# nvidia-cosmos/cosmos-curate

Hardware: AMD Instinct MI355X
Metric: clips/sec + embedded frames/sec, 1080p30 H.264, 1/2/4/8 MI355X (higher is better)
Workload: dtype bf16; 1 GPU; split_pipeline 1xMI355X: HIP NV12->RGB/resize + CLIP-ViT-B/32 MFMA bf16 (decode seam excluded: no librocdecode in image); model=vit_b32, frames_per_clip=21, src=1080p30 NV12 in HBM, resolution=224, parallelism=dp1

## Files before the change

cosmos_curate_amd/csrc/cc_gemm.hip:

```cpp

#include <hip/hip_runtime.h>

#include "cc_common.hpp"
#include "cc_gemm_plan.hpp"
#include "cc_timing.hpp"

namespace {

typedef __attribute__((ext_vector_type(8))) __bf16 bf16x8;
typedef __attribute__((ext_vector_type(4))) float f32x4;

constexpr int BM = cc::GEMM_T128, BN = cc::GEMM_T128, BK = cc::GEMM_BK;
constexpr int WM = 64, WN = 64;
constexpr int FRAG = 16;
constexpr int MFR = WM / FRAG;
constexpr int NFR = WN / FRAG;

__device__ __forceinline__ unsigned short f32_to_bf16_rne(float v) {
  union {
    float f;
    unsigned int u;
  } cv{v};
  unsigned int lsb = (cv.u >> 16) & 1;
  return (unsigned short)((cv.u + 0x7fffu + lsb) >> 16);
}

template <int ACT>
__device__ __forceinline__ float cc_act(float v) {
  if constexpr (ACT == 1)
    return v * __builtin_amdgcn_rcpf(1.0f + __expf(-1.702f * v));
  if constexpr (ACT == 2) {
    float z = 0.7978845608028654f * (v + 0.044715f * v * v * v);
    float t = 1.0f - 2.0f * __builtin_amdgcn_rcpf(__expf(2.0f * z) + 1.0f);
    return 0.5f * v * (1.0f + t);
  }
  if constexpr (ACT == 3)
    return 0.5f * v * (1.0f + erff(v * 0.70710678f));
  return v;
}

__device__ __forceinline__ int xcd_remap(int orig, int nwg) {
  int q = nwg >> 3, r = nwg & 7;
  int xcd = orig & 7, lid = orig >> 3;
  return (xcd < r ? xcd * (q + 1) : r * (q + 1) + (xcd - r) * q) + lid;
}

template <int CHUNKS>
__device__ __forceinline__ void stage_rows(const __bf16* __restrict__ src,
                                           long ld, long row0, long row_limit,
                                           long k0, __bf16* lds_base,
                                           int lane) {
  const int lrow8 = lane >> 3;
  const int slot = lane & 7;
  const int gk16 = slot ^ lrow8;
#pragma unroll
  for (int j = 0; j < CHUNKS; j++) {
    long grow = row0 + j * 8 + lrow8;
    grow = grow < 0 ? 0 : (grow >= row_limit ? row_limit - 1 : grow);
    const __bf16* gptr = src + grow * ld + k0 + (long)gk16 * 8;
    __builtin_amdgcn_global_load_lds(
        (const __attribute__((address_space(1))) unsigned int*)gptr,
        (__attribute__((address_space(3))) unsigned int*)(lds_base + j * 8 * BK),
        16, 0, 0);
  }
}

__device__ __forceinline__ bf16x8 frag_read(const __bf16* tile, int row,
                                            int k16) {
  int slot = k16 ^ (row & 7);
  return *(const bf16x8*)(tile + (long)row * BK + slot * 8);
}

template <int ACT, bool HAS_BIAS, bool HAS_RES, bool LN_IN>
__global__ __launch_bounds__(256, 2) void k_gemm_bf16(
    const __bf16* __restrict__ A, const __bf16* __restrict__ B,
    void* __restrict__ C, const float* __restrict__ bias,
    const __bf16* __restrict__ residual, long M, long N, long K, long lda,
    long ldr, int c_is_bf16, int nbx, int nwg, int do_remap,
    const float* __restrict__ colsum, const float2* __restrict__ murstd) {
  __shared__ __bf16 lds[2 * (BM + BN) * BK];
#define AS(b) (lds + (b) * (BM * BK))
#define BS(b) (lds + 2 * (BM * BK) + (b) * (BN * BK))

  const int tid = threadIdx.x;
  const int lane = tid & 63;
  const int wid = tid >> 6;
  const int waveM = wid >> 1, waveN = wid & 1;

  int orig = blockIdx.x;
  if (do_remap) orig = xcd_remap(orig, nwg);
  const long bm = (long)(orig / nbx) * BM;
  const long bn = (long)(orig % nbx) * BN;

  const long arow0 = bm + 32 * wid;
  const long brow0 = bn + 32 * wid;

  f32x4 acc[MFR][NFR] = {};

  const long KT = K / BK;
  stage_rows<4>(A, lda, arow0, M, 0, AS(0) + 32 * wid * BK, lane);
  stage_rows<4>(B, K, brow0, N, 0, BS(0) + 32 * wid * BK, lane);

  const int arow_frag = waveM * WM + (lane & 15);
  const int brow_frag = waveN * WN + (lane & 15);
  int buf = 0;
  for (long kt = 0; kt < KT; ++kt) {
    asm volatile("s_waitcnt vmcnt(0)" ::: "memory");
    __syncthreads();
    const __bf16* At = AS(buf);
    const __bf16* Bt = BS(buf);
    bf16x8 afrag[2][MFR], bfrag[2][NFR];
#pragma unroll
    for (int g = 0; g < 2; g++) {
      const int k16 = (g << 2) + (lane >> 4);
#pragma unroll
      for (int m = 0; m < MFR; m++)
        afrag[g][m] = frag_read(At, arow_frag + m * FRAG, k16);
#pragma unroll
      for (int n = 0; n < NFR; n++)
        bfrag[g][n] = frag_read(Bt, brow_frag + n * FRAG, k16);
    }
    if (kt + 1 < KT) {
      const long k0 = (kt + 1) * BK;
      stage_rows<4>(A, lda, arow0, M, k0, AS(buf ^ 1) + 32 * wid * BK, lane);
      stage_rows<4>(B, K, brow0, N, k0, BS(buf ^ 1) + 32 * wid * BK, lane);
    }
#pragma unroll
    for (int g = 0; g < 2; g++)
#pragma unroll
      for (int m = 0; m < MFR; m++)
#pragma unroll
        for (int n = 0; n < NFR; n++)
          acc[m][n] = __builtin_amdgcn_mfma_f32_16x16x32_bf16(
              afrag[g][m], bfrag[g][n], acc[m][n], 0, 0, 0);
    buf ^= 1;
  }

  const long crow_base = bm + waveM * WM + 4 * (lane >> 4);
  const long ccol_base = bn + waveN * WN + (lane & 15);
  const bool interior = (bm + BM <= M) && (bn + BN <= N);
  if (interior) {
#pragma unroll
    for (int m = 0; m < MFR; m++) {
      float2 mr[4] = {};
      if constexpr (LN_IN) {
#pragma unroll
        for (int r = 0; r < 4; r++) mr[r] = murstd[crow_base + m * FRAG + r];
      }
#pragma unroll
      for (int n = 0; n < NFR; n++) {
        const long col = ccol_base + n * FRAG;
        float bval = 0.0f;
        if constexpr (HAS_BIAS) bval = bias[col];
        if constexpr (LN_IN) {
          const float sval = colsum[col];
#pragma unroll
          for (int r = 0; r < 4; r++)
            acc[m][n][r] = mr[r].y * (acc[m][n][r] - mr[r].x * sval);
        }
        float rv[4];
        if constexpr (HAS_RES) {
#pragma unroll
          for (int r = 0; r < 4; r++)
            rv[r] = (float)residual[(crow_base + m * FRAG + r) * ldr + col];
        }
#pragma unroll
        for (int r = 0; r < 4; r++) {
          const long row = crow_base + m * FRAG + r;
          float v = cc_act<ACT>(acc[m][n][r] + bval);
          if constexpr (HAS_RES) v += rv[r];
          if (c_is_bf16)
            ((unsigned short*)C)[row * N + col] = f32_to_bf16_rne(v);
          else
            ((float*)C)[row * N + col] = v;
        }
      }
    }
    return;
  }
#pragma unroll
  for (int m = 0; m < MFR; m++) {
#pragma unroll
    for (int n = 0; n < NFR; n++) {
      const long col = ccol_base + n * FRAG;
      if (col >= N) continue;
      float bval = 0.0f;
      if constexpr (HAS_BIAS) bval = bias[col];
#pragma unroll
      for (int r = 0; r < 4; r++) {
        const long row = crow_base + m * FRAG + r;
        if (row >= M) continue;
        if constexpr (LN_IN) {
          const float2 mr = murstd[row];
          acc[m][n][r] = mr.y * (acc[m][n][r] - mr.x * colsum[col]);
        }
        float v = cc_act<ACT>(acc[m][n][r] + bval);
        if constexpr (HAS_RES) v += (float)residual[row * ldr + col];
        if (c_is_bf16)
          ((unsigned short*)C)[row * N + col] = f32_to_bf16_rne(v);
        else
          ((float*)C)[row * N + col] = v;
      }
    }
  }
#undef AS
#undef BS
}

constexpr int BM2 = cc::GEMM_T256, BN2 = cc::GEMM_T256;
constexpr int WM2 = 128, WN2 = 64;
constexpr int MFR2 = WM2 / FRAG;
constexpr int NFR2 = WN2 / FRAG;

constexpr int LN_TAB = BM2 * 4;

template <int CTRL>
__device__ __forceinline__ float dpp_add(float v) {
  const int o = __builtin_amdgcn_update_dpp(0, __builtin_bit_cast(int, v),
                                            CTRL, 0xf, 0xf, false);
  return v + __builtin_bit_cast(float, o);
}
__device__ __forceinline__ float sum8(float v) {
  return dpp_add<0x141>(dpp_add<0x4e>(dpp_add<0xb1>(v)));
}

template <int ACT, bool HAS_BIAS, bool HAS_RES, bool EPI_STAGED, bool LN_IN,
          bool STATS>
__global__ __launch_bounds__(512, 1) void k_gemm_bf16_t256(
    const __bf16* __restrict__ A, const __bf16* __restrict__ B,
    void* __restrict__ C, const float* __restrict__ bias,
    const __bf16* __restrict__ residual, long M, long N, long K,
    int c_is_bf16, int nbx, int nwg, int order_mode,
    const float* __restrict__ colsum, const float2* __restrict__ murstd,
    float2* __restrict__ stats) {
  static_assert(!STATS || HAS_RES, "the stats epilogue is the residual one");
  __shared__ __bf16 lds[2 * (BM2 + BN2) * BK + (LN_IN ? 2 * LN_TAB : 0)];
#define LNTAB(b) ((float*)(lds + 2 * (BM2 + BN2) * BK + (b) * LN_TAB))
#define STAGE_LN2(b)                                                        \
  do {                                                                      \
    if constexpr (LN_IN) {                                                  \
      const long r = bm + (tid >> 1);                                       \
      const float* g = (const float*)(murstd + (r < M ? r : M - 1)) +       \
                       (tid & 1);                                           \
      __builtin_amdgcn_global_load_lds(                                     \
          (const __attribute__((address_space(1))) unsigned int*)g,         \
          (__attribute__((address_space(3))) unsigned int*)(LNTAB(b) +      \
                                                            wid * 64),      \
          4, 0, 0);                                                         \
    }                                                                       \
  } while (0)
#define A2T(b) (lds + (b) * (BM2 * BK))
#define B2T(b) (lds + 2 * (BM2 * BK) + (b) * (BN2 * BK))
  const int tid = threadIdx.x;
  const int lane = tid & 63;
  const int wid = tid >> 6;
  const int waveM = wid >> 2, waveN = wid & 3;
  const long KT = K / BK;
  const long srow = wid * 16;
  const int arow_base = waveM * WM2 + (lane & 15);
  const int brow_base = waveN * WN2 + (lane & 15);
  bf16x8 bfragT[NFR2][2];
  bf16x8 afrag[2][2];

#define STAGE_A2(t, h)                                                      \
  stage_rows<2>(A, K, bm + (h) * 128 + srow, M, (t) * BK,                   \
                A2T((t) & 1) + ((h) * 128 + srow) * BK, lane)
#define STAGE_B2(t, h)                                                      \
  stage_rows<2>(B, K, bn + (h) * 128 + srow, N, (t) * BK,                   \
                B2T((t) & 1) + ((h) * 128 + srow) * BK, lane)

  const int tiles = (nwg + (int)gridDim.x - 1) / (int)gridDim.x;
  long bm, bn;
  {
    int orig = (int)blockIdx.x;
    if (order_mode == 1) orig = xcd_remap(orig, nwg);
    bm = (long)(orig / nbx) * BM2;
    bn = (long)(orig % nbx) * BN2;
  }
  STAGE_LN2(0);
  STAGE_A2(0, 0);
  STAGE_A2(0, 1);
  STAGE_B2(0, 0);
  STAGE_B2(0, 1);
  STAGE_B2(1, 0);
  STAGE_B2(1, 1);

  for (int rep = 0; rep < tiles; rep++) {
    if ((int)blockIdx.x + rep * (int)gridDim.x >= nwg) break;
    f32x4 acc[MFR2][NFR2] = {};
    asm volatile("s_waitcnt vmcnt(0)" ::: "memory");
    __builtin_amdgcn_s_barrier();

#define PHASE_MFMA2(q)                                                      \
  do {                                                                      \
    asm volatile("s_waitcnt lgkmcnt(0)" ::: "memory");                      \
     \
     \
     \
     \
     \
     \
     \
     \
     \
     \
    __builtin_amdgcn_sched_group_barrier(0x8 , 2, 0);               \
    _Pragma("unroll") for (int gi = 0; gi < 6; gi++) {                      \
      __builtin_amdgcn_sched_group_barrier(0x100 , 1, 0);        \
      __builtin_amdgcn_sched_group_barrier(0x8 , 2, 0);             \
      __builtin_amdgcn_sched_group_barrier(0x10 , 1, 0);            \
    }                                                                       \
    _Pragma("unroll") for (int g = 0; g < 2; g++) {                         \
      _Pragma("unroll") for (int m = 0; m < 2; m++) {                       \
        _Pragma("unroll") for (int n = 0; n < NFR2; n++) {                  \
          acc[2 * (q) + m][n] = __builtin_amdgcn_mfma_f32_16x16x32_bf16(    \
              afrag[m][g], bfragT[n][g], acc[2 * (q) + m][n], 0, 0, 0);     \
        }                                                                   \
      }                                                                     \
    }                                                                       \
  } while (0)

#define READ_A2(At, q)                                                      \
  _Pragma("unroll") for (int g = 0; g < 2; g++) {                           \
    const int k16 = (g << 2) + (lane >> 4);                                 \
    _Pragma("unroll") for (int m = 0; m < 2; m++) afrag[m][g] =             \
        frag_read(At, arow_base + (q) * 32 + m * FRAG, k16);                \
  }

#define READ_B2(Bt)                                                         \
  _Pragma("unroll") for (int g = 0; g < 2; g++) {                           \
    const int k16 = (g << 2) + (lane >> 4);                                 \
    _Pragma("unroll") for (int n = 0; n < NFR2; n++) bfragT[n][g] =         \
        frag_read(Bt, brow_base + n * FRAG, k16);                           \
  }

#define KTILE2(t)                                                           \
  do {                                                                      \
    const __bf16* At = A2T((t) & 1);                                        \
    const __bf16* Bt = B2T((t) & 1);                                        \
     \
     \
     \
    asm volatile("s_waitcnt vmcnt(4)" ::: "memory");                        \
    READ_B2(Bt);                                                            \
    READ_A2(At, 0);                                                         \
    if ((t) + 1 < KT) STAGE_A2((t) + 1, 0);                                 \
    __builtin_amdgcn_s_barrier();                                           \
    PHASE_MFMA2(0);                                                         \
    READ_A2(At, 1);                                                         \
    if ((t) + 1 < KT) STAGE_A2((t) + 1, 1);                                 \
    __builtin_amdgcn_s_barrier();                                           \
    PHASE_MFMA2(1);                                                         \
    READ_A2(At, 2);                                                         \
    __builtin_amdgcn_s_barrier();                                           \
    PHASE_MFMA2(2);                                                         \
    READ_A2(At, 3);                                                         \
     \
     \
     \
     \
     \
     \
     \
     \
     \
     \
     \
     \
    if ((t) + 2 < KT) {                                                     \
      STAGE_B2((t) + 2, 0);                                                 \
      STAGE_B2((t) + 2, 1);                                                 \
       \
       \
       \
       \
       \
       \
       \
       \
       \
      asm volatile("s_waitcnt vmcnt(4)" ::: "memory");                      \
    } else {                                                                \
      asm volatile("s_waitcnt vmcnt(0)" ::: "memory");      \
    }                                                                       \
    __builtin_amdgcn_s_barrier();                                           \
    PHASE_MFMA2(3);                                                         \
  } while (0)

    for (long it = 0; it < KT / 2; ++it) {
      KTILE2(2 * it);
      KTILE2(2 * it + 1);
    }

    const long ebm = bm, ebn = bn;
    __builtin_amdgcn_s_barrier();
    if (rep + 1 < tiles &&
        (int)blockIdx.x + (rep + 1) * (int)gridDim.x < nwg) {
      int orig = (int)blockIdx.x + (rep + 1) * (int)gridDim.x;
      if (order_mode == 1) orig = xcd_remap(orig, nwg);
      bm = (long)(orig / nbx) * BM2;
      bn = (long)(orig % nbx) * BN2;
      STAGE_LN2((rep + 1) & 1);
      STAGE_A2(0, 0);
      STAGE_A2(0, 1);
      STAGE_B2(0, 0);
      STAGE_B2(0, 1);
      STAGE_B2(1, 0);
      STAGE_B2(1, 1);
    }

    const long crow_base = ebm + waveM * WM2 + 4 * (lane >> 4);
    const long ccol_base = ebn + waveN * WN2 + (lane & 15);
    if ((c_is_bf16 && EPI_STAGED) || LN_IN || STATS) {
      __bf16* slice = A2T(1) + wid * 2048;
      const long wrow0 = ebm + waveM * WM2;
      const long wcol0 = ebn + waveN * WN2;
      float bhoist[NFR2] = {};
      if constexpr (HAS_BIAS) {
#pragma unroll
        for (int n = 0; n < NFR2; n++) {
          const long col = ccol_base + n * FRAG;
          bhoist[n] = (col < N) ? bias[col] : 0.0f;
        }
      }
      float shoist[NFR2] = {};
      if constexpr (LN_IN) {
#pragma unroll
        for (int n = 0; n < NFR2; n++) {
          const long col = ccol_base + n * FRAG;
          shoist[n] = (col < N) ? colsum[col] : 0.0f;
        }
      }
#pragma unroll
      for (int p = 0; p < 4; p++) {
#pragma unroll
        for (int mm = 0; mm < 2; mm++) {
          const int m = 2 * p + mm;
          float2 mr[4] = {};
          if constexpr (LN_IN) {
            const float2* t = (const float2*)LNTAB(rep & 1) + waveM * WM2 +
                              m * FRAG + 4 * (lane >> 4);
#pragma unroll
            for (int r = 0; r < 4; r++) mr[r] = t[r];
          }
#pragma unroll
          for (int n = 0; n < NFR2; n++) {
            const float bval = bhoist[n];
            const int lrow_b = mm * 16 + 4 * (lane >> 4);
            const int lcol = n * FRAG + (lane & 15);
#pragma unroll
            for (int r = 0; r < 4; r++) {
              if constexpr (LN_IN)
                acc[m][n][r] = mr[r].y * (acc[m][n][r] - mr[r].x * shoist[n]);
              float v = cc_act<ACT>(acc[m][n][r] + bval);
              *(unsigned short*)(slice + (lrow_b + r) * 64 + lcol) =
                  f32_to_bf16_rne(v);
            }
          }
        }
        asm volatile("s_waitcnt lgkmcnt(0)" ::: "memory");
#pragma unroll
        for (int i = 0; i < 4; i++) {
          const int elem = i * 512 + lane * 8;
          const int lrow = elem >> 6;
          const int lcol8 = elem & 63;
          const long grow = wrow0 + p * 32 + lrow;
          const long gcol = wcol0 + lcol8;
          if constexpr (STATS) {
            const bool ok = grow < M && gcol < N;
            float s = 0.0f, ss = 0.0f;
            if (ok) {
              bf16x8 v8 = *(const bf16x8*)(slice + elem);
              const bf16x8 r8 = *(const bf16x8*)(residual + grow * N + gcol);
#pragma unroll
              for (int e = 0; e < 8; e++) {
                v8[e] = (__bf16)((float)v8[e] + (float)r8[e]);
                const float f = (float)v8[e];
                s += f;
                ss += f * f;
              }
              *(bf16x8*)((__bf16*)C + grow * N + gcol) = v8;
            }
            s = sum8(s);
            ss = sum8(ss);
            if (ok && (lane & 7) == 0)
              stats[grow * (N >> 6) + (gcol >> 6)] = make_float2(s, ss);
            continue;
          }
          if (grow >= M || gcol >= N) continue;
          bf16x8 v8 = *(const bf16x8*)(slice + elem);
          if constexpr (HAS_RES) {
            const bf16x8 r8 =
                *(const bf16x8*)(residual + grow * N + gcol);
#pragma unroll
            for (int e = 0; e < 8; e++)
              v8[e] = (__bf16)((float)v8[e] + (float)r8[e]);
          }
          *(bf16x8*)((__bf16*)C + grow * N + gcol) = v8;
        }
      }
    } else {
      const bool interior = (ebm + BM2 <= M) && (ebn + BN2 <= N);
      float bhoist2[NFR2] = {};
      if constexpr (HAS_BIAS) {
#pragma unroll
        for (int n = 0; n < NFR2; n++) {
          const long col = ccol_base + n * FRAG;
          bhoist2[n] = (interior || col < N) ? bias[col] : 0.0f;
        }
      }
#pragma unroll
      for (int m = 0; m < MFR2; m++) {
#pragma unroll
        for (int n = 0; n < NFR2; n++) {
          const long col = ccol_base + n * FRAG;
          if (!interior && col >= N) continue;
          const float bval = bhoist2[n];
#pragma unroll
          for (int r = 0; r < 4; r++) {
            const long row = crow_base + m * FRAG + r;
            if (!interior && row >= M) continue;
            float v = cc_act<ACT>(acc[m][n][r] + bval);
            if constexpr (HAS_RES) v += (float)residual[row * N + col];
            if (c_is_bf16)
              ((unsigned short*)C)[row * N + col] = f32_to_bf16_rne(v);
            else
              ((float*)C)[row * N + col] = v;
          }
        }
      }
    }
  }
#undef LNTAB
#undef STAGE_LN2
#undef A2T
#undef B2T
#undef STAGE_A2
#undef STAGE_B2
#undef PHASE_MFMA2
#undef READ_A2
#undef READ_B2
#undef KTILE2
}

struct GemmArgs {
  const __bf16 *A, *B;
  void* C;
  const float* bias;
  const __bf16* residual;
  long M, N, K, lda, ldr;
  int c_is_bf16;
  hipStream_t stream;
  const float* colsum = nullptr;
  const float2* murstd = nullptr;
  float2* stats = nullptr;
};

template <int ACT, bool HB, bool HR, bool LN = false, bool ST = false>
void gemm_run(const cc_gemm_plan_info& p, const GemmArgs& g) {
  const int nwg = p.tiles_x * p.tiles_y;
  if (p.body == cc::GEMM_T256)
    hipLaunchKernelGGL(
        (k_gemm_bf16_t256<ACT, HB, HR, ACT != 0 || HB || HR, LN, ST>),
        dim3(p.grid), dim3(p.block), 0, g.stream, g.A, g.B, g.C, g.bias,
        g.residual, g.M, g.N, g.K, g.c_is_bf16, p.tiles_x, nwg, p.xcd_remap,
        g.colsum, g.murstd, g.stats);
  else
    hipLaunchKernelGGL((k_gemm_bf16<ACT, HB, HR, LN>), dim3(p.grid),
                       dim3(p.block), 0, g.stream, g.A, g.B, g.C, g.bias,
                       g.residual, g.M, g.N, g.K, g.lda, g.ldr, g.c_is_bf16,
                       p.tiles_x, nwg, p.xcd_remap, g.colsum, g.murstd);
}

using GemmRunFn = void (*)(const cc_gemm_plan_info&, const GemmArgs&);
constexpr GemmRunFn kGemmRun[4][2][2] = {
    {{gemm_run<0, false, false>, gemm_run<0, false, true>},
     {gemm_run<0, true, false>, gemm_run<0, true, true>}},
    {{gemm_run<1, false, false>, gemm_run<1, false, true>},
     {gemm_run<1, true, false>, gemm_run<1, true, true>}},
    {{gemm_run<2, false, false>, gemm_run<2, false, true>},
     {gemm_run<2, true, false>, gemm_run<2, true, true>}},
    {{nullptr, nullptr}, {gemm_run<3, true, false>, nullptr}}};
constexpr GemmRunFn kGemmRunLn[4] = {
    gemm_run<0, true, false, true>, gemm_run<1, true, false, true>,
    gemm_run<2, true, false, true>, gemm_run<3, true, false, true>};

int check_act(int act) {
  if (act < 0 || act > 3)
    return cc::set_error(CC_ERR_INVALID,
                         "gemm act must be 0 (none), 1 (quick-gelu), 2 "
                         "(tanh-gelu) or 3 (erf-gelu), got %d", act);
  return CC_OK;
}

int gemm_launch(const void* A, int64_t lda, const void* B, void* C, int64_t M,
                int64_t N, int64_t K, const float* bias, int c_dtype, int act,
                const void* residual, int64_t ldr, uint64_t stream) {
  if (!A || !B || !C) return cc::set_error(CC_ERR_INVALID, "bad gemm args");
  if (int rc = check_act(act)) return rc;
  const GemmRunFn run = kGemmRun[act][bias != nullptr][residual != nullptr];
  if (!run)
    return cc::set_error(CC_ERR_UNSUPPORTED,
                         "gemm act %d is instantiated with a bias and "
                         "without a residual only", act);
  cc_gemm_plan_info plan;
  if (int rc = cc::gemm_plan(M, N, K, lda, ldr, bias != nullptr, act,
                             residual != nullptr, cc::gemm_env_knobs(), &plan))
    return rc;
  const GemmArgs args{(const __bf16*)A, (const __bf16*)B, C, bias,
                      (const __bf16*)residual, (long)M, (long)N, (long)K,
                      (long)lda, (long)ldr, c_dtype == 1 ? 1 : 0,
                      (hipStream_t)stream};
  return cc::timed_launch("gemm_bf16", stream, [&] { run(plan, args); });
}

int gemm_norm_in(bool rms, const void* A, int64_t row_step, const void* stats,
                 void* murstd, const void* Wfold, const float* colsum,
                 const float* cbias, void* C, int64_t M, int64_t N, int64_t K,
                 int act, float eps, uint64_t stream) {
  if (!A || !stats || !murstd || !Wfold || !colsum || !cbias || !C ||
      row_step <= 0)
    return cc::set_error(CC_ERR_INVALID, "bad gemm_ln args");
  if (int rc = check_act(act)) return rc;
  if (!cc::ln_h_supported(K))
    return cc::set_error(CC_ERR_UNSUPPORTED,
                         "gemm_ln: no LayerNorm statistics at K %lld",
                         (long long)K);
  cc_gemm_plan_info plan;
  if (int rc = cc::gemm_plan(M, N, K, row_step * K, N, true, act, false,
                             cc::gemm_env_knobs(), &plan))
    return rc;
  if (int rc = rms ? cc_rms_finalize(stats, M, K, row_step, eps, murstd, stream)
                   : cc_ln_finalize(stats, M, K, row_step, eps, murstd, stream))
    return rc;
  GemmArgs args{(const __bf16*)A, (const __bf16*)Wfold, C, cbias, nullptr,
                (long)M, (long)N, (long)K, (long)(row_step * K), (long)N, 1,
                (hipStream_t)stream};
  args.colsum = colsum;
  args.murstd = (const float2*)murstd;
  return cc::timed_launch("gemm_bf16", stream, [&] {
    kGemmRunLn[act](plan, args);
  });
}
}

extern "C" int cc_gemm_plan(int64_t M, int64_t N, int64_t K, int64_t lda,
                            int64_t ldr, int has_bias, int act,
                            int has_residual, cc_gemm_plan_info* out) {
  if (!out) return cc::set_error(CC_ERR_INVALID, "cc_gemm_plan: null out");
  return cc::gemm_plan(M, N, K, lda, ldr, has_bias != 0, act,
                       has_residual != 0, cc::GemmKnobs{}, out);
}

extern "C" int cc_gemm_bf16_ex(const void* A, const void* B, void* C,
                               int64_t M, int64_t N, int64_t K,
                               const float* bias, int c_dtype, int act,
                               const void* residual, uint64_t stream) {
  return gemm_launch(A, K, B, C, M, N, K, bias, c_dtype, act, residual, N,
                     stream);
}

extern "C" int cc_gemm_bf16_strided(const void* A, int64_t lda, const void* B,
                                    void* C, int64_t M, int64_t N, int64_t K,
                                    const float* bias, int c_dtype, int act,
                                    const void* residual, int64_t ldr,
                                    uint64_t stream) {
  return gemm_launch(A, lda, B, C, M, N, K, bias, c_dtype, act, residual, ldr,
                     stream);
}

extern "C" int cc_gemm_bf16(const void* A, const void* B, void* C, int64_t M,
                            int64_t N, int64_t K, const float* bias,
                            int c_dtype, uint64_t stream) {
  return cc_gemm_bf16_ex(A, B, C, M, N, K, bias, c_dtype, 0, nullptr, stream);
}

extern "C" int cc_gemm_bf16_res_stats(const void* A, const void* B, void* C,
                                      int64_t M, int64_t N, int64_t K,
                                      const float* bias, const void* residual,
                                      void* stats, uint64_t stream) {
  if (!A || !B || !C || !bias || !residual || !stats)
    return cc::set_error(CC_ERR_INVALID, "bad gemm_res_stats args");
  if (!cc::ln_h_supported(N))
    return cc::set_error(CC_ERR_UNSUPPORTED,
                         "gemm_res_stats: no LayerNorm statistics at N %lld",
                         (long long)N);
  cc_gemm_plan_info plan;
  if (int rc = cc::gemm_plan(M, N, K, K, N, true, 0, true,
                             cc::gemm_env_knobs(), &plan))
    return rc;
  GemmArgs args{(const __bf16*)A, (const __bf16*)B, C, bias,
                (const __bf16*)residual, (long)M, (long)N, (long)K, (long)K,
                (long)N, 1, (hipStream_t)stream};
  if (plan.body == cc::GEMM_T256 && cc::gemm_env_knobs().fuse_stats) {
    args.stats = (float2*)stats;
    return cc::timed_launch("gemm_bf16", stream, [&] {
      gemm_run<0, true, true, false, true>(plan, args);
    });
  }
  if (int rc = cc::timed_launch("gemm_bf16", stream, [&] {
        gemm_run<0, true, true>(plan, args);
      }))
    return rc;
  return cc_ln_stats_bf16(C, M, N, stats, stream);
}

extern "C" int cc_gemm_bf16_ln(const void* A, int64_t row_step,
                               const void* stats, void* murstd,
                               const void* Wfold, const float* colsum,
                               const float* cbias, void* C, int64_t M,
                               int64_t N, int64_t K, int act, float eps,
                               uint64_t stream) {
  return gemm_norm_in(false, A, row_step, stats, murstd, Wfold, colsum, cbias,
                      C, M, N, K, act, eps, stream);
}

extern "C" int cc_gemm_bf16_rms(const void* A, int64_t row_step,
                                const void* stats, void* murstd,
                                const void* Wfold, const float* colsum,
                                const float* cbias, void* C, int64_t M,
                                int64_t N, int64_t K, int act, float eps,
                                uint64_t stream) {
  return gemm_norm_in(true, A, row_step, stats, murstd, Wfold, colsum, cbias,
                      C, M, N, K, act, eps, stream);
}
```

Measured before the change: 4967 clips/s.

## Prefetch residual and column tables, overlap epilogue stores with next-tile prologue

Reworks the persistent 256-tile GEMM epilogue. Residual rows are prefetched into registers with inline-asm loads before the next tile's prologue loads are issued. Bias and colsum are staged into LDS through global_load_lds, and output and stats writes go through buffer stores whose out-of-bounds offsets drop writes instead of branching. The point is to stop draining vmcnt(0) between tiles, so epilogue stores and the next tile's loads overlap. In exchange it depends on hand-counted vmcnt values that must match the exact number of loads and stores in flight, which is fragile and can silently break correctness.

```diff
diff --git a/cosmos_curate_amd/csrc/cc_gemm.hip b/cosmos_curate_amd/csrc/cc_gemm.hip
--- a/cosmos_curate_amd/csrc/cc_gemm.hip
+++ b/cosmos_curate_amd/csrc/cc_gemm.hip
@@ -213,6 +213,27 @@
 constexpr int NFR2 = WN2 / FRAG;
 
 constexpr int LN_TAB = BM2 * 4;
+constexpr int COL_TAB = BN2 * 4;
+
+typedef __attribute__((ext_vector_type(4))) unsigned int u32x4;
+typedef __attribute__((ext_vector_type(2))) unsigned int u32x2;
+__device__ __forceinline__ void load16_uncounted(u32x4& dst, const void* base,
+                                                 unsigned byte_off) {
+  asm volatile("s_nop 4\n\tglobal_load_dwordx4 %0, %1, %2"
+               : "=v"(dst)
+               : "v"(byte_off), "s"(base)
+               : "memory");
+}
+template <int CNT_NEXT, int CNT_LAST>
+__device__ __forceinline__ void res_wait(bool has_next, u32x4 (&r)[4]) {
+  static_assert(CNT_NEXT >= CNT_LAST && CNT_LAST >= 0 && CNT_NEXT < 64,
+                "vmcnt is a 6-bit field");
+  if (has_next)
+    asm volatile("s_waitcnt vmcnt(%0)" ::"n"(CNT_NEXT) : "memory");
+  else
+    asm volatile("s_waitcnt vmcnt(%0)" ::"n"(CNT_LAST) : "memory");
+  asm volatile("" : "+v"(r[0]), "+v"(r[1]), "+v"(r[2]), "+v"(r[3])::"memory");
+}
 
 template <int CTRL>
 __device__ __forceinline__ float dpp_add(float v) {
@@ -234,7 +255,26 @@
     const float* __restrict__ colsum, const float2* __restrict__ murstd,
     float2* __restrict__ stats) {
   static_assert(!STATS || HAS_RES, "the stats epilogue is the residual one");
-  __shared__ __bf16 lds[2 * (BM2 + BN2) * BK + (LN_IN ? 2 * LN_TAB : 0)];
+  static_assert(!LN_IN || HAS_BIAS, "the folded norm always carries a bias");
+  constexpr bool COLTAB = HAS_BIAS;
+  __shared__ __bf16 lds[2 * (BM2 + BN2) * BK + (LN_IN ? 2 * LN_TAB : 0) +
+                        (COLTAB ? 2 * COL_TAB : 0)];
+#define COLTAB_AT(b)                                                        \
+  ((float*)(lds + 2 * (BM2 + BN2) * BK + (LN_IN ? 2 * LN_TAB : 0) +         \
+            (b) * COL_TAB))
+#define STAGE_COL2(b)                                                       \
+  do {                                                                      \
+    if constexpr (COLTAB) {                                                 \
+      const long c = bn + (wid & 3) * 64 + lane;                            \
+      const float* g = ((LN_IN && wid >= 4) ? colsum : bias) +              \
+                       (c < N ? c : N - 1);                                 \
+      __builtin_amdgcn_global_load_lds(                                     \
+          (const __attribute__((address_space(1))) unsigned int*)g,         \
+          (__attribute__((address_space(3))) unsigned int*)(COLTAB_AT(b) +  \
+                                                            wid * 64),      \
+          4, 0, 0);                                                         \
+    }                                                                       \
+  } while (0)
 #define LNTAB(b) ((float*)(lds + 2 * (BM2 + BN2) * BK + (b) * LN_TAB))
 #define STAGE_LN2(b)                                                        \
   do {                                                                      \
@@ -278,6 +318,7 @@
     bn = (long)(orig % nbx) * BN2;
   }
   STAGE_LN2(0);
+  STAGE_COL2(0);
   STAGE_A2(0, 0);
   STAGE_A2(0, 1);
   STAGE_B2(0, 0);
@@ -285,10 +326,20 @@
   STAGE_B2(1, 0);
   STAGE_B2(1, 1);
 
+  constexpr int PRO_LOADS = 12 + (LN_IN ? 1 : 0) + (COLTAB ? 1 : 0);
+  constexpr int PASS_STORES = STATS ? 8 : 4;
+  const bool staged = (c_is_bf16 && EPI_STAGED) || LN_IN || STATS;
+  asm volatile("s_waitcnt vmcnt(0)" ::: "memory");
+
   for (int rep = 0; rep < tiles; rep++) {
     if ((int)blockIdx.x + rep * (int)gridDim.x >= nwg) break;
     f32x4 acc[MFR2][NFR2] = {};
-    asm volatile("s_waitcnt vmcnt(0)" ::: "memory");
+    if (rep > 0) {
+      if (staged)
+        asm volatile("s_waitcnt vmcnt(%0)" ::"n"(4 * PASS_STORES) : "memory");
+      else
+        asm volatile("s_waitcnt vmcnt(0)" ::: "memory");
+    }
     __builtin_amdgcn_s_barrier();
 
 #define PHASE_MFMA2(q)                                                      \
@@ -341,7 +392,11 @@
      \
      \
      \
-    asm volatile("s_waitcnt vmcnt(4)" ::: "memory");                        \
+     \
+     \
+     \
+    asm volatile("s_waitcnt vmcnt(%0)" ::"n"(4 + 4 * PASS_STORES)           \
+                 : "memory");                                               \
     READ_B2(Bt);                                                            \
     READ_A2(At, 0);                                                         \
     if ((t) + 1 < KT) STAGE_A2((t) + 1, 0);                                 \
@@ -394,43 +449,77 @@
 
     const long ebm = bm, ebn = bn;
     __builtin_amdgcn_s_barrier();
-    if (rep + 1 < tiles &&
-        (int)blockIdx.x + (rep + 1) * (int)gridDim.x < nwg) {
-      int orig = (int)blockIdx.x + (rep + 1) * (int)gridDim.x;
-      if (order_mode == 1) orig = xcd_remap(orig, nwg);
-      bm = (long)(orig / nbx) * BM2;
-      bn = (long)(orig % nbx) * BN2;
-      STAGE_LN2((rep + 1) & 1);
-      STAGE_A2(0, 0);
-      STAGE_A2(0, 1);
-      STAGE_B2(0, 0);
-      STAGE_B2(0, 1);
-      STAGE_B2(1, 0);
-      STAGE_B2(1, 1);
-    }
+    int tid_e = tid;
+    asm volatile("" : "+v"(tid_e));
+    {
+    const int tid = tid_e, lane = tid_e & 63, wid = tid_e >> 6;
+    const int waveM = wid >> 2, waveN = wid & 3;
+    const long srow = wid * 16;
+    const bool has_next = rep + 1 < tiles &&
+                          (int)blockIdx.x + (rep + 1) * (int)gridDim.x < nwg;
+    const int n32 = (int)N;
+    const int tile_rows = (int)((M - ebm) < BM2 ? (M - ebm) : BM2);
+    int row_off = (waveM * WM2 + (lane >> 3)) * n32;
+    asm volatile("" : "+v"(row_off));
+    const int col_abs = (int)ebn + waveN * WN2 + (lane & 7) * 8;
+    u32x4 resq[4][4];
+    auto issue_res = [&](int p) {
+      if constexpr (HAS_RES) {
+        const __bf16* rbase = residual + ebm * N;
+        const int last_row = (tile_rows - 1) * n32;
+        const int col = col_abs < n32 ? col_abs : n32 - 8;
+#pragma unroll
+        for (int i = 0; i < 4; i++) {
+          const int ro = row_off + (p * 32 + i * 8) * n32;
+          load16_uncounted(resq[p][i], rbase,
+                           ((ro < last_row ? ro : last_row) + col) * 2);
+        }
+      }
+    };
+    auto next_prologue = [&] {
+      if (has_next) {
+        int orig = (int)blockIdx.x + (rep + 1) * (int)gridDim.x;
+        if (order_mode == 1) orig = xcd_remap(orig, nwg);
+        bm = (long)(orig / nbx) * BM2;
+        bn = (long)(orig % nbx) * BN2;
+        STAGE_LN2((rep + 1) & 1);
+        STAGE_COL2((rep + 1) & 1);
+        STAGE_A2(0, 0);
+        STAGE_A2(0, 1);
+        STAGE_B2(0, 0);
+        STAGE_B2(0, 1);
+        STAGE_B2(1, 0);
+        STAGE_B2(1, 1);
+      }
+    };
 
     const long crow_base = ebm + waveM * WM2 + 4 * (lane >> 4);
     const long ccol_base = ebn + waveN * WN2 + (lane & 15);
-    if ((c_is_bf16 && EPI_STAGED) || LN_IN || STATS) {
+    if (staged) {
+      issue_res(0);
+      issue_res(1);
+      issue_res(2);
+      next_prologue();
       __bf16* slice = A2T(1) + wid * 2048;
-      const long wrow0 = ebm + waveM * WM2;
-      const long wcol0 = ebn + waveN * WN2;
       float bhoist[NFR2] = {};
-      if constexpr (HAS_BIAS) {
+      float shoist[NFR2] = {};
+      if constexpr (COLTAB) {
+        const float* ct = COLTAB_AT(rep & 1) + waveN * WN2 + (lane & 15);
 #pragma unroll
         for (int n = 0; n < NFR2; n++) {
-          const long col = ccol_base + n * FRAG;
-          bhoist[n] = (col < N) ? bias[col] : 0.0f;
+          bhoist[n] = ct[n * FRAG];
+          if constexpr (LN_IN) shoist[n] = ct[BN2 + n * FRAG];
         }
       }
-      float shoist[NFR2] = {};
-      if constexpr (LN_IN) {
-#pragma unroll
-        for (int n = 0; n < NFR2; n++) {
-          const long col = ccol_base + n * FRAG;
-          shoist[n] = (col < N) ? colsum[col] : 0.0f;
-        }
-      }
+      constexpr unsigned OOB = 0x80000000u;
+      const __amdgpu_buffer_rsrc_t c_rsrc = __builtin_amdgcn_make_buffer_rsrc(
+          (__bf16*)C + ebm * N, 0, tile_rows * n32 * 2, 0x00020000);
+      __amdgpu_buffer_rsrc_t s_rsrc = c_rsrc;
+      if constexpr (STATS)
+        s_rsrc = __builtin_amdgcn_make_buffer_rsrc(
+            stats + ebm * (N >> 6), 0, tile_rows * (n32 >> 6) * 8, 0x00020000);
+#define RES_WAIT(p, cnt)                                                    \
+  res_wait<(cnt) + PRO_LOADS, (cnt)>(has_next, resq[p])
 #pragma unroll
       for (int p = 0; p < 4; p++) {
 #pragma unroll
@@ -438,10 +527,11 @@
           const int m = 2 * p + mm;
           float2 mr[4] = {};
           if constexpr (LN_IN) {
-            const float2* t = (const float2*)LNTAB(rep & 1) + waveM * WM2 +
-                              m * FRAG + 4 * (lane >> 4);
-#pragma unroll
-            for (int r = 0; r < 4; r++) mr[r] = t[r];
+            const float* t = LNTAB(rep & 1) +
+                             2 * (waveM * WM2 + m * FRAG + 4 * (lane >> 4));
+#pragma unroll
+            for (int r = 0; r < 4; r++)
+              mr[r] = make_float2(t[2 * r], t[2 * r + 1]);
           }
 #pragma unroll
           for (int n = 0; n < NFR2; n++) {
@@ -458,56 +548,64 @@
             }
           }
         }
+        if constexpr (HAS_RES) {
+          if (p == 0) {
+            issue_res(3);
+            RES_WAIT(0, 12);
+          } else if (p == 1) {
+            RES_WAIT(1, PASS_STORES + 8);
+          } else if (p == 2) {
+            RES_WAIT(2, 2 * PASS_STORES + 4);
+          } else {
+            res_wait<3 * PASS_STORES, 3 * PASS_STORES>(has_next, resq[3]);
+          }
+        }
         asm volatile("s_waitcnt lgkmcnt(0)" ::: "memory");
 #pragma unroll
         for (int i = 0; i < 4; i++) {
           const int elem = i * 512 + lane * 8;
-          const int lrow = elem >> 6;
-          const int lcol8 = elem & 63;
-          const long grow = wrow0 + p * 32 + lrow;
-          const long gcol = wcol0 + lcol8;
-          if constexpr (STATS) {
-            const bool ok = grow < M && gcol < N;
-            float s = 0.0f, ss = 0.0f;
-            if (ok) {
-              bf16x8 v8 = *(const bf16x8*)(slice + elem);
-              const bf16x8 r8 = *(const bf16x8*)(residual + grow * N + gcol);
-#pragma unroll
-              for (int e = 0; e < 8; e++) {
-                v8[e] = (__bf16)((float)v8[e] + (float)r8[e]);
+          const int ro = row_off + (p * 32 + i * 8) * n32;
+          const bool col_ok = col_abs < n32;
+          const unsigned c_off = col_ok ? (unsigned)(ro + col_abs) * 2 : OOB;
+          bf16x8 v8 = *(const bf16x8*)(slice + elem);
+          float s = 0.0f, ss = 0.0f;
+          if constexpr (HAS_RES) {
+            const bf16x8 r8 = __builtin_bit_cast(bf16x8, resq[p][i]);
+#pragma unroll
+            for (int e = 0; e < 8; e++) {
+              v8[e] = (__bf16)((float)v8[e] + (float)r8[e]);
+              if constexpr (STATS) {
                 const float f = (float)v8[e];
                 s += f;
                 ss += f * f;
               }
-              *(bf16x8*)((__bf16*)C + grow * N + gcol) = v8;
             }
+          }
+          __builtin_amdgcn_raw_buffer_store_b128(
+              __builtin_bit_cast(u32x4, v8), c_rsrc, (int)c_off, 0, 0);
+          if constexpr (STATS) {
             s = sum8(s);
             ss = sum8(ss);
-            if (ok && (lane & 7) == 0)
-              stats[grow * (N >> 6) + (gcol >> 6)] = make_float2(s, ss);
-            continue;
+            const unsigned s_off =
+                (col_ok && (lane & 7) == 0)
+                    ? (unsigned)((ro + col_abs) >> 6) * 8
+                    : OOB;
+            u32x2 st;
+            st[0] = __builtin_bit_cast(unsigned, s);
+            st[1] = __builtin_bit_cast(unsigned, ss);
+            __builtin_amdgcn_raw_buffer_store_b64(st, s_rsrc, (int)s_off, 0, 0);
           }
-          if (grow >= M || gcol >= N) continue;
-          bf16x8 v8 = *(const bf16x8*)(slice + elem);
-          if constexpr (HAS_RES) {
-            const bf16x8 r8 =
-                *(const bf16x8*)(residual + grow * N + gcol);
-#pragma unroll
-            for (int e = 0; e < 8; e++)
-              v8[e] = (__bf16)((float)v8[e] + (float)r8[e]);
-          }
-          *(bf16x8*)((__bf16*)C + grow * N + gcol) = v8;
         }
       }
+#undef RES_WAIT
     } else {
+      next_prologue();
       const bool interior = (ebm + BM2 <= M) && (ebn + BN2 <= N);
       float bhoist2[NFR2] = {};
       if constexpr (HAS_BIAS) {
-#pragma unroll
-        for (int n = 0; n < NFR2; n++) {
-          const long col = ccol_base + n * FRAG;
-          bhoist2[n] = (interior || col < N) ? bias[col] : 0.0f;
-        }
+        const float* ct = COLTAB_AT(rep & 1) + waveN * WN2 + (lane & 15);
+#pragma unroll
+        for (int n = 0; n < NFR2; n++) bhoist2[n] = ct[n * FRAG];
       }
 #pragma unroll
       for (int m = 0; m < MFR2; m++) {
@@ -530,9 +628,12 @@
         }
       }
     }
+    }
   }
 #undef LNTAB
 #undef STAGE_LN2
+#undef COLTAB_AT
+#undef STAGE_COL2
 #undef A2T
 #undef B2T
 #undef STAGE_A2
```

New measurement: 5140 clips/s, median of 6. 1.03x the previous value.
